# google-deepmind/open_spiel

Hardware: AMD Instinct MI355X
Metric: env-steps/sec (batched LegalActions+ApplyAction+status, connect_four) (higher is better)
Workload: dtype u64; 1 GPU; connect_four fused LegalActions+ApplyAction+status, 2^20 states/GPU, seed 0x5EED; states_per_gpu=1048576, parallelism=1 independent shard(s), no collective

## Files before the change

### open_spiel_amd/csrc/osg_c4_step.h

```cpp
#ifndef OSG_C4_STEP_H_
#define OSG_C4_STEP_H_

#include "osg_common.h"

namespace osg {

OSG_HD uint64_t c4_fours(uint64_t b) {
  uint64_t hit, m;
  m = b & (b >> 1); hit = m & (m >> 2);
  m = b & (b >> 7); hit |= m & (m >> 14);
  m = b & (b >> 6); hit |= m & (m >> 12);
  m = b & (b >> 8); hit |= m & (m >> 16);
  return hit;
}

OSG_HD uint32_t c4_open_columns(uint32_t all_lo, uint32_t all_hi) {
  const uint32_t tl = (~all_lo >> 5) & 0x00204081u;
  const uint32_t th = (~all_hi >> 1) & 0x00004081u;
  const uint32_t ml = tl * ((1u << 21) | (1u << 15) | (1u << 9) | (1u << 3));
  const uint32_t mh = th * ((1u << 14) | (1u << 8) | (1u << 2));
  return ((ml >> 21) & 0xFu) | (((mh >> 14) & 0x7u) << 4);
}

OSG_HD uint32_t c4_fused_step(uint64_t& x, uint64_t& o, uint32_t a) {
  const uint32_t flags = static_cast<uint32_t>(x >> 56);
  const uint64_t X = x & ((1ull << 56) - 1ull), O = o;
  const uint64_t all = X | O;
  const uint32_t stones = static_cast<uint32_t>(__builtin_popcountll(all));
  const uint32_t mover = stones & 1u;
  const bool valid = a < 7u;
  const uint32_t sh = valid ? a * 7u : 0u;
  const uint64_t cell = (all + (1ull << sh)) & (0x3Full << sh);
  const bool apply = valid & ((flags & 1u) == 0u) & (cell != 0ull);
  const uint64_t put = apply ? cell : 0ull;
  const uint64_t to_x = mover ? 0ull : ~0ull;
  const uint64_t nx = X | (put & to_x), no = O | (put & ~to_x);
  const uint64_t b = mover ? no : nx;
  const bool win = c4_fours(b) != 0ull;
  const uint32_t stones_after = stones + (apply ? 1u : 0u);
  const bool done = win | (stones_after == 42u);
  const uint32_t fresh = done ? (((win ? mover : 2u) << 1) | 1u) : 0u;
  const uint32_t nflags = apply ? fresh : flags;
  const uint64_t nall = nx | no;
  const uint32_t open = c4_open_columns(static_cast<uint32_t>(nall), static_cast<uint32_t>(nall >> 32));
  const bool over = (nflags & 1u) != 0u;
  const uint32_t st_run = (stones_after & 1u) + 1u;
  const uint32_t st_over = 0x80u | (nflags >> 1);
  const uint32_t st = (over ? st_over : st_run) | (((a != 0xFFu) & !apply) ? 0x40u : 0u);
  x = nx | (static_cast<uint64_t>(nflags) << 56);
  o = no;
  return (over ? 0u : open) | (st << 8);
}

}
#endif
```

### open_spiel_amd/csrc/osg_step.hip

```cpp
#include "osg_batch_internal.h"
#include "osg_c4_step.h"
#include "osg_ttt_step.h"

namespace {

OSG_D uint8_t encode_status(bool terminal, bool illegal, int cur, int outcome) {
  uint8_t v = illegal ? 0x40 : 0;
  if (terminal) return v | 0x80 | static_cast<uint8_t>(outcome & 7);
  return v | static_cast<uint8_t>((cur + 1) & 15);
}
template <class G> struct has_fused_step : std::false_type {};
template <int R, int C, int K, class BB> struct has_fused_step<C4T<R, C, K, BB>> : std::integral_constant<bool, !C4T<R, C, K, BB>::kStored> {};
template <class G, typename MaskT>
__global__ void __launch_bounds__(kBlock)
k_step(typename G::Params p, const typename G::word_t* src, typename G::word_t* dst, int64_t n,
       const uint8_t* actions, MaskT* mask_out, int mask_elems, uint8_t* status) {
  int64_t i = static_cast<int64_t>(blockIdx.x) * kBlock + threadIdx.x;
  if (i >= n) return;
  typename G::State s = G::load(p, src, n, i);
  int a = actions[i];
  if constexpr (has_fused_step<G>::value) {
    bool illegal_f, term_f;
    int outcome_f;
    const uint32_t open = G::fused_step(p, s, a, illegal_f, term_f, outcome_f);
    G::store(p, dst, n, i, s);
    if (sizeof(MaskT) < 4) {
      mask_out[i] = static_cast<MaskT>(open);
    } else {
#pragma unroll
      for (int w = 0; w < G::kMaskW; ++w)
        if (w < mask_elems) mask_out[i * mask_elems + w] = static_cast<MaskT>(w == 0 ? open : 0u);
    }
    status[i] = encode_status(term_f, illegal_f, term_f ? 0 : (G::plies(s) & 1), term_f ? outcome_f : 0);
    return;
  }
  bool illegal = false;
  if (a != 0xFF) {
    auto before = G::legal(p, s);
    if (a < 32 * G::kMaskW && before.test(a)) G::apply(p, s, a); else illegal = true;
  }
  G::store(p, dst, n, i, s);
  bool term = G::terminal(p, s);
  auto after = G::legal(p, s);
  if (sizeof(MaskT) < 4) {
    mask_out[i] = static_cast<MaskT>(after.w[0]);
  } else {
#pragma unroll
    for (int w = 0; w < G::kMaskW; ++w)
      if (w < mask_elems) mask_out[i * mask_elems + w] = static_cast<MaskT>(after.w[w]);
  }
  status[i] = encode_status(term, illegal, term ? 0 : G::current_player(p, s), term ? G::outcome_code(p, s) : 0);
}

template <class G, typename MaskT, int V, int W>
__global__ void __launch_bounds__(kBlock)
k_step_vec(typename G::Params p, const typename G::word_t* src, typename G::word_t* dst, int64_t n,
           const uint8_t* __restrict__ actions, MaskT* __restrict__ mask_out, uint8_t* __restrict__ status) {
  using word_t = typename G::word_t;
  typedef word_t wvec __attribute__((ext_vector_type(V)));
  typedef uint8_t bvec __attribute__((ext_vector_type(V)));
  typedef MaskT mvec __attribute__((ext_vector_type(V)));
  const int64_t i = (static_cast<int64_t>(blockIdx.x) * kBlock + threadIdx.x) * V;
  if (i >= n) return;
  word_t tmp[W * V];
#pragma unroll
  for (int w = 0; w < W; ++w) {
    const wvec v = *reinterpret_cast<const wvec*>(src + w * n + i);
#pragma unroll
    for (int j = 0; j < V; ++j) tmp[w * V + j] = v[j];
  }
  const bvec av = *reinterpret_cast<const bvec*>(actions + i);
  bvec sv;
  mvec mv;
#pragma unroll
  for (int j = 0; j < V; ++j) {
    if constexpr (std::is_same<G, Ttt>::value) {
      const uint32_t r = ttt_fused_step(tmp[j], av[j]);
      mv[j] = static_cast<MaskT>(r & 0xFFFFu);
      sv[j] = static_cast<uint8_t>(r >> 16);
      continue;
    }
    typename G::State s = G::load(p, tmp, V, j);
    const int a = av[j];
    bool illegal = false;
    if (a != 0xFF) {
      const auto before = G::legal(p, s);
      if (a < 32 * G::kMaskW && before.test(a)) G::apply(p, s, a); else illegal = true;
    }
    G::store(p, tmp, V, j, s);
    const bool term = G::terminal(p, s);
    const auto after = G::legal(p, s);
    mv[j] = static_cast<MaskT>(after.w[0]);
    sv[j] = encode_status(term, illegal, term ? 0 : G::current_player(p, s), term ? G::outcome_code(p, s) : 0);
  }
#pragma unroll
  for (int w = 0; w < W; ++w) {
    wvec v;
#pragma unroll
    for (int j = 0; j < V; ++j) v[j] = tmp[w * V + j];
    __builtin_nontemporal_store(v, reinterpret_cast<wvec*>(dst + w * n + i));
  }
  __builtin_nontemporal_store(mv, reinterpret_cast<mvec*>(mask_out + i));
  __builtin_nontemporal_store(sv, reinterpret_cast<bvec*>(status + i));
}

template <int NW, int V, bool kNt, bool kMask = true, bool kFold = false>
__global__ void __launch_bounds__(kBlock)
k_step_hexvec(typename HexT<NW>::Params p, const uint32_t* src, uint32_t* dst, int64_t n,
              const uint8_t* __restrict__ actions, uint32_t* __restrict__ mask_out, uint8_t* __restrict__ status) {
  using G = HexT<NW>;
  constexpr int W = kFold ? 4 * NW : 4 * NW + 1;
  typedef uint32_t wvec __attribute__((ext_vector_type(V)));
  typedef uint8_t bvec __attribute__((ext_vector_type(V)));
  const int64_t i = (static_cast<int64_t>(blockIdx.x) * kBlock + threadIdx.x) * V;
  if (i >= n) return;
  uint32_t tmp[W * V];
#pragma unroll
  for (int w = 0; w < W; ++w) {
    const wvec v = *reinterpret_cast<const wvec*>(src + w * n + i);
#pragma unroll
    for (int j = 0; j < V; ++j) tmp[w * V + j] = v[j];
  }
  const bvec av = *reinterpret_cast<const bvec*>(actions + i);
  uint32_t mk[NW * V];
  bvec sv;
#pragma unroll
  for (int j = 0; j < V; ++j) {
    typename G::State s = G::template load_as<kFold>(tmp, V, j);
    const int a = av[j];
    bool illegal = false;
    if (a != 0xFF) {
      const auto before = G::legal(p, s);
      if (a < 32 * G::kMaskW && before.test(a)) G::apply(p, s, a); else illegal = true;
    }
    G::template store_as<kFold>(tmp, V, j, s);
    const bool term = G::terminal(p, s);
    if constexpr (kMask) {
      const auto after = G::legal(p, s);
#pragma unroll
      for (int w = 0; w < NW; ++w) mk[j * NW + w] = after.w[w];
    }
    sv[j] = encode_status(term, illegal, term ? 0 : G::current_player(p, s), term ? G::outcome_code(p, s) : 0);
  }
#pragma unroll
  for (int w = 0; w < W; ++w) {
    wvec v;
#pragma unroll
    for (int j = 0; j < V; ++j) v[j] = tmp[w * V + j];
    if constexpr (kNt) __builtin_nontemporal_store(v, reinterpret_cast<wvec*>(dst + w * n + i));
    else *reinterpret_cast<wvec*>(dst + w * n + i) = v;
  }
  if constexpr (kMask) {
#pragma unroll
    for (int k = 0; k < NW; ++k) {
      wvec v;
#pragma unroll
      for (int j = 0; j < V; ++j) v[j] = mk[k * V + j];
      if constexpr (kNt) __builtin_nontemporal_store(v, reinterpret_cast<wvec*>(mask_out + i * NW) + k);
      else reinterpret_cast<wvec*>(mask_out + i * NW)[k] = v;
    }
  }
  if constexpr (kNt) __builtin_nontemporal_store(sv, reinterpret_cast<bvec*>(status + i));
  else *reinterpret_cast<bvec*>(status + i) = sv;
}

constexpr int kC4StepBlock = 128;
template <class G>
__global__ void __launch_bounds__(kC4StepBlock)
k_step_c4x2(typename G::Params p, const uint64_t* src, uint64_t* dst, int64_t n,
            const uint8_t* __restrict__ actions, uint8_t* __restrict__ mask_out, uint8_t* __restrict__ status) {
  const int64_t pair = static_cast<int64_t>(blockIdx.x) * kC4StepBlock + threadIdx.x;
  const int64_t i = pair * 2;
  if (i >= n) return;
  const ulonglong2 xs = *reinterpret_cast<const ulonglong2*>(src + i);
  const ulonglong2 os = *reinterpret_cast<const ulonglong2*>(src + n + i);
  const uint32_t a2 = *reinterpret_cast<const uint16_t*>(actions + i);
  uint64_t x[2] = {xs.x, xs.y}, o[2] = {os.x, os.y};
  uint32_t m2 = 0, s2 = 0;
#pragma unroll
  for (int j = 0; j < 2; ++j) {
    typename G::State s = G::unpack(x[j], o[j]);
    const int a = (a2 >> (8 * j)) & 0xFF;
    bool term = G::terminal(p, s);
    bool illegal = false;
    if (a != 0xFF) {
      if (!term && G::column_has_room(p, s, a)) {
        G::apply(p, s, a);
        term = G::terminal(p, s);
      } else {
        illegal = true;
      }
    }
    const uint32_t open = G::open_columns(p, s);
    const int to_move = G::plies(s) & 1;
    x[j] = G::pack0(s);
    o[j] = s.o;
    m2 |= (term ? 0u : (open & 0xFFu)) << (8 * j);
    s2 |= static_cast<uint32_t>(encode_status(term, illegal, to_move, term ? G::outcome_code(p, s) : 0)) << (8 * j);
  }
  *reinterpret_cast<ulonglong2*>(dst + i) = make_ulonglong2(x[0], x[1]);
  *reinterpret_cast<ulonglong2*>(dst + n + i) = make_ulonglong2(o[0], o[1]);
  *reinterpret_cast<uint16_t*>(mask_out + i) = static_cast<uint16_t>(m2);
  *reinterpret_cast<uint16_t*>(status + i) = static_cast<uint16_t>(s2);
}

__global__ void __launch_bounds__(kC4StepBlock)
k_step_c4std(const uint64_t* src, uint64_t* dst, int64_t n, const uint8_t* __restrict__ actions,
             uint8_t* __restrict__ mask_out, uint8_t* __restrict__ status) {
  const int64_t i = static_cast<int64_t>(blockIdx.x) * kC4StepBlock + threadIdx.x;
  if (i >= n) return;
  uint64_t x = src[i], o = src[n + i];
  const uint32_t r = c4_fused_step(x, o, actions[i]);
  __builtin_nontemporal_store(x, dst + i);
  __builtin_nontemporal_store(o, dst + n + i);
  __builtin_nontemporal_store(static_cast<uint8_t>(r), mask_out + i);
  __builtin_nontemporal_store(static_cast<uint8_t>(r >> 8), status + i);
}

__global__ void __launch_bounds__(kC4StepBlock)
k_step_c4std2(const uint64_t* src, uint64_t* dst, int64_t n, const uint8_t* __restrict__ actions,
              uint8_t* __restrict__ mask_out, uint8_t* __restrict__ status) {
  const int64_t i = (static_cast<int64_t>(blockIdx.x) * kC4StepBlock + threadIdx.x) * 2;
  if (i >= n) return;
  typedef uint64_t u64x2 __attribute__((ext_vector_type(2)));
  typedef uint8_t u8x2 __attribute__((ext_vector_type(2)));
  const u64x2 xs = *reinterpret_cast<const u64x2*>(src + i), os = *reinterpret_cast<const u64x2*>(src + n + i);
  const u8x2 av = *reinterpret_cast<const u8x2*>(actions + i);
  uint64_t x0 = xs.x, x1 = xs.y, o0 = os.x, o1 = os.y;
  const uint32_t r0 = c4_fused_step(x0, o0, av.x), r1 = c4_fused_step(x1, o1, av.y);
  u64x2 xo, oo;
  xo.x = x0; xo.y = x1; oo.x = o0; oo.y = o1;
  u8x2 mo, so;
  mo.x = static_cast<uint8_t>(r0); mo.y = static_cast<uint8_t>(r1);
  so.x = static_cast<uint8_t>(r0 >> 8); so.y = static_cast<uint8_t>(r1 >> 8);
  __builtin_nontemporal_store(xo, reinterpret_cast<u64x2*>(dst + i));
  __builtin_nontemporal_store(oo, reinterpret_cast<u64x2*>(dst + n + i));
  __builtin_nontemporal_store(mo, reinterpret_cast<u8x2*>(mask_out + i));
  __builtin_nontemporal_store(so, reinterpret_cast<u8x2*>(status + i));
}

}

extern "C" {

int osg_step(const osg_batch* src, osg_batch* dst, const uint8_t* d_actions, void* d_mask, uint8_t* d_status) {
  if (!same_game(dst, src) || dst->n != src->n) return set_error(OSG_ERR_INVALID, "osg_step: shape mismatch");
  if (src->spec.desc.num_distinct_actions > 255)
    return set_error(OSG_ERR_UNSUPPORTED, "osg_step: action ids travel as one byte here (0xFF = skip); games with more than 255 "
                                          "actions (hex above 15 x 15) step through osg_apply / osg_env_step (32-bit actions)");
  osg_ctx* ctx = dst->ctx;
  const int cmb = src->spec.desc.compact_mask_bytes;
  const int W = src->spec.desc.mask_words;
  const int64_t n = src->n;
  if (!d_mask && !(src->spec.desc.game_kind == kHex && W == src->spec.hex_nw && W <= 4))
    return set_error(OSG_ERR_UNSUPPORTED, "osg_step: d_mask may be NULL only for hex boards of up to 128 cells (there the successor's "
                                          "mask is ~occupied of the record written); every other game's mask comes from the step itself");
  const bool planes16 = ((reinterpret_cast<uintptr_t>(src->words()) | reinterpret_cast<uintptr_t>(dst->words())) & 15u) == 0;
  if (planes16 && src->spec.desc.game_kind == kC4 && src->spec.c4_std && (n & 1) == 0 &&
      ((reinterpret_cast<uintptr_t>(d_actions) | reinterpret_cast<uintptr_t>(d_mask) | reinterpret_cast<uintptr_t>(d_status)) & 1u) == 0) {
    k_step_c4std2<<<dim3(static_cast<unsigned>((n / 2 + kC4StepBlock - 1) / kC4StepBlock)), dim3(kC4StepBlock), 0, ctx->stream>>>(
        static_cast<const uint64_t*>(src->words()), static_cast<uint64_t*>(dst->words()), n, d_actions,
        static_cast<uint8_t*>(d_mask), d_status);
    OSG_HIP(hipGetLastError());
    return OSG_OK;
  }
  if (src->spec.desc.game_kind == kC4 && src->spec.c4_std) {
    k_step_c4std<<<dim3(static_cast<unsigned>((n + kC4StepBlock - 1) / kC4StepBlock)), dim3(kC4StepBlock), 0, ctx->stream>>>(
        static_cast<const uint64_t*>(src->words()), static_cast<uint64_t*>(dst->words()), n, d_actions,
        static_cast<uint8_t*>(d_mask), d_status);
    OSG_HIP(hipGetLastError());
    return OSG_OK;
  }
  const bool aligned2 = ((reinterpret_cast<uintptr_t>(d_actions) | reinterpret_cast<uintptr_t>(d_mask) |
                          reinterpret_cast<uintptr_t>(d_status)) & 1u) == 0;
  if (planes16 && src->spec.desc.game_kind == kC4 && !src->spec.c4_wide && (n & 1) == 0 && aligned2) {
    const int64_t pairs = n / 2;
    k_step_c4x2<C4><<<dim3(static_cast<unsigned>((pairs + kC4StepBlock - 1) / kC4StepBlock)), dim3(kC4StepBlock), 0, ctx->stream>>>(
        src->spec.c4, static_cast<const uint64_t*>(src->words()), static_cast<uint64_t*>(dst->words()), n, d_actions,
        static_cast<uint8_t*>(d_mask), d_status);
    OSG_HIP(hipGetLastError());
    return OSG_OK;
  }
  const uintptr_t side = reinterpret_cast<uintptr_t>(d_actions) | reinterpret_cast<uintptr_t>(d_mask) | reinterpret_cast<uintptr_t>(d_status);
  const int kind = src->spec.desc.game_kind;
  if (planes16 && kind == kTtt && (n & 3) == 0 && (side & 7u) == 0 && cmb == 2) {
    k_step_vec<Ttt, uint16_t, 4, 1><<<dim3(grid_for(n / 4)), dim3(kBlock), 0, ctx->stream>>>(
        src->spec.ttt, static_cast<const uint32_t*>(src->words()), static_cast<uint32_t*>(dst->words()), n, d_actions,
        static_cast<uint16_t*>(d_mask), d_status);
    OSG_HIP(hipGetLastError());
    return OSG_OK;
  }
  if (planes16 && kind == kKuhn && (n & 1) == 0 && (side & 1u) == 0 && cmb == 1) {
    k_step_vec<Kuhn, uint8_t, 2, 1><<<dim3(grid_for(n / 2)), dim3(kBlock), 0, ctx->stream>>>(
        src->spec.kuhn, static_cast<const uint64_t*>(src->words()), static_cast<uint64_t*>(dst->words()), n, d_actions,
        static_cast<uint8_t*>(d_mask), d_status);
    OSG_HIP(hipGetLastError());
    return OSG_OK;
  }
  if (planes16 && kind == kLeduc && !src->spec.leduc_big && n >= (int64_t{1} << 22) && (n & 1) == 0 && (side & 1u) == 0 && cmb == 1) {
    k_step_vec<Leduc, uint8_t, 2, 2><<<dim3(grid_for(n / 2)), dim3(kBlock), 0, ctx->stream>>>(
        src->spec.leduc, static_cast<const uint64_t*>(src->words()), static_cast<uint64_t*>(dst->words()), n, d_actions,
        static_cast<uint8_t*>(d_mask), d_status);
    OSG_HIP(hipGetLastError());
    return OSG_OK;
  }
  if (kind == kHex && (cmb == 4 * W || !d_mask) && W == src->spec.hex_nw && W <= 4) {
    int v = 2, nt = n >= (int64_t{1} << 22) ? 1 : 0;
    if (const char* e = std::getenv("OSG_HEX_STEP")) {
      int ev = 0, ent = 0;
      if (std::sscanf(e, "%d:%d", &ev, &ent) == 2 && (ev == 1 || ev == 2)) { v = ev; nt = ent ? 1 : 0; }
    }
    while (v > 1 && ((n % v) != 0 || (side & static_cast<uintptr_t>(v - 1)) != 0 ||
                     (reinterpret_cast<uintptr_t>(d_mask) & static_cast<uintptr_t>(4 * v - 1)) != 0 || !planes16))
      v >>= 1;
    if (v > 1) {
      const auto* s32 = static_cast<const uint32_t*>(src->words());
      auto* d32 = static_cast<uint32_t*>(dst->words());
      auto* m32 = static_cast<uint32_t*>(d_mask);
      if (int rc = for_hex(src->spec, [&](auto nw, const auto& P) -> int {
            constexpr int NW = decltype(nw)::value;
            if constexpr (NW <= 4) {
              return with_bool(src->spec.hex_fold, [&](auto fold) {
                return with_bool(nt != 0, [&](auto ntv) {
                  return with_bool(m32 != nullptr, [&](auto mask) {
                    k_step_hexvec<NW, 2, decltype(ntv)::value, decltype(mask)::value, decltype(fold)::value>
                        <<<dim3(grid_for(n / 2)), dim3(kBlock), 0, ctx->stream>>>(P, s32, d32, n, d_actions, m32, d_status);
                    return OSG_OK;
                  });
                });
              });
            }
            return OSG_OK;
          })) return rc;
      OSG_HIP(hipGetLastError());
      return OSG_OK;
    }
  }
  if (!d_mask)
    return set_error(OSG_ERR_UNSUPPORTED, "osg_step: d_mask may be NULL only for hex boards of up to 128 cells stepped two states per "
                                          "thread (an even batch, 2-byte aligned side arrays): there the successor's mask is ~occupied "
                                          "of the record written; every other game's mask is computed by the step itself");
  const auto step = [&](auto m, int mask_stride) {
    using M = decltype(m);
    return for_game(src->spec, [&](auto g, const auto& P) {
      using G = typename decltype(g)::type;
      k_step<G, M><<<dim3(grid_for(n)), dim3(kBlock), 0, ctx->stream>>>(P, static_cast<const typename G::word_t*>(src->words()),
          static_cast<typename G::word_t*>(dst->words()), n, d_actions,
          static_cast<M*>(d_mask), mask_stride, d_status);
      return OSG_OK;
    });
  };
  if (int rc = cmb == 1 ? step(uint8_t{}, 1) : cmb == 2 ? step(uint16_t{}, 1) : step(uint32_t{}, W)) return rc;
  OSG_HIP(hipGetLastError());
  return OSG_OK;
}

}
```

Baseline: 228.2 billion env-steps/s.

## Step two connect-four states per thread with packed 16-bit high-word bitboard math

Adds a paired fused-step path that splits each 64-bit bitboard into 32-bit halves and packs the two states' small upper words into one register. Four-in-a-row detection then runs on the packed word using packed 16-bit shifts, alignbit funnels, perm and bitop3, and the mask and status bytes are extracted with perm. A fallback to the scalar path handles boards whose high bits exceed 16, and an asm hint keeps the kernel pointers in scalar registers. The goal is fewer 64-bit ALU instructions in a kernel that may be memory-bound, at the cost of more complex code and a divergent branch.

```diff
diff --git a/open_spiel_amd/csrc/osg_c4_step.h b/open_spiel_amd/csrc/osg_c4_step.h
--- a/open_spiel_amd/csrc/osg_c4_step.h
+++ b/open_spiel_amd/csrc/osg_c4_step.h
@@ -52,5 +52,134 @@
   return (over ? 0u : open) | (st << 8);
 }
 
+
+typedef uint16_t c4_u16x2 __attribute__((ext_vector_type(2)));
+
+OSG_HD uint32_t c4_pk_shr(uint32_t p, uint32_t d) {
+  const c4_u16x2 v = __builtin_bit_cast(c4_u16x2, p) >> static_cast<uint16_t>(d);
+  return __builtin_bit_cast(uint32_t, v);
+}
+OSG_HD uint32_t c4_funnel(uint32_t hi, uint32_t lo, uint32_t d) {
+#if defined(__HIP_DEVICE_COMPILE__)
+  return __builtin_amdgcn_alignbit(hi, lo, d);
+#else
+  return (lo >> d) | (hi << (32u - d));
+#endif
+}
+OSG_HD uint32_t c4_pack16(uint32_t lo, uint32_t hi) {
+#if defined(__HIP_DEVICE_COMPILE__)
+  return __builtin_amdgcn_perm(hi, lo, 0x05040100u);
+#else
+  return (lo & 0xFFFFu) | (hi << 16);
+#endif
+}
+OSG_HD uint32_t c4_upper16(uint32_t lo, uint32_t hi) {
+#if defined(__HIP_DEVICE_COMPILE__)
+  return __builtin_amdgcn_perm(hi, lo, 0x07060302u);
+#else
+  return (lo >> 16) | (hi & 0xFFFF0000u);
+#endif
+}
+constexpr uint32_t kA = 0xF0u, kB = 0xCCu, kC = 0xAAu;
+template <uint32_t T> OSG_HD uint32_t c4_op3(uint32_t a, uint32_t b, uint32_t c) {
+#if defined(__HIP_DEVICE_COMPILE__)
+  return __builtin_amdgcn_bitop3_b32(a, b, c, T & 0xFFu);
+#else
+  uint32_t r = 0u;
+  for (uint32_t k = 0; k < 8u; ++k)
+    if ((T >> k) & 1u) r |= ((k & 4u) ? a : ~a) & ((k & 2u) ? b : ~b) & ((k & 1u) ? c : ~c);
+  return r;
+#endif
+}
+OSG_HD uint32_t c4_select(uint32_t m, uint32_t a, uint32_t b) { return c4_op3<(kA & kB) | (~kA & kC)>(m, a, b); }
+OSG_HD uint32_t c4_andn_or(uint32_t a, uint32_t b, uint32_t c) { return c4_op3<(kA & ~kB) | kC>(a, b, c); }
+
+struct c4_placement {
+  uint32_t put_lo, put_hi, tx, stones_after, flags;
+  bool apply;
+};
+OSG_HD c4_placement c4_place(uint32_t x_lo, uint32_t x_hi_raw, uint32_t o_lo, uint32_t o_hi, uint32_t a) {
+  c4_placement r;
+  r.flags = x_hi_raw >> 24;
+  const uint32_t all_lo = x_lo | o_lo, all_hi = (x_hi_raw & 0xFFFFFFu) | o_hi;
+  const uint32_t stones = static_cast<uint32_t>(__builtin_popcount(all_lo) + __builtin_popcount(all_hi));
+  const bool ok = (a < 7u) & ((r.flags & 1u) == 0u);
+  const uint32_t sh = (a * 7u) & 63u;
+  const uint32_t col = static_cast<uint32_t>(((static_cast<uint64_t>(all_hi) << 32) | all_lo) >> sh);
+  const uint32_t cell = (col + 1u) & (ok ? 0x3Fu : 0u);
+  const uint64_t put = static_cast<uint64_t>(cell) << sh;
+  r.apply = cell != 0u;
+  r.put_lo = static_cast<uint32_t>(put);
+  r.put_hi = static_cast<uint32_t>(put >> 32);
+  r.tx = (stones & 1u) - 1u;
+  r.stones_after = stones + (r.apply ? 1u : 0u);
+  return r;
+}
+
+OSG_HD uint32_t c4_finish(const c4_placement& p, bool win, uint32_t open, uint32_t a, uint32_t& nflags) {
+  const uint32_t mover = (p.tx & 1u) ^ 1u;
+  const bool done = win | (p.stones_after == 42u);
+  const uint32_t fresh = done ? (((win ? mover : 2u) << 1) | 1u) : 0u;
+  nflags = p.apply ? fresh : p.flags;
+  const bool over = (nflags & 1u) != 0u;
+  const uint32_t st_run = (p.stones_after & 1u) + 1u;
+  const uint32_t st_over = 0x80u | (nflags >> 1);
+  const uint32_t st = (over ? st_over : st_run) | (((a != 0xFFu) & !p.apply) ? 0x40u : 0u);
+  return (over ? 0u : open) | (st << 8);
+}
+
+template <uint32_t D>
+OSG_HD void c4_fours_dir(uint32_t b0, uint32_t b1, uint32_t bp, uint32_t bh1, uint32_t& h0, uint32_t& h1, uint32_t& hp) {
+  const uint32_t mp = bp & c4_pk_shr(bp, D);
+  const uint32_t m0 = b0 & c4_funnel(bp, b0, D), m1 = b1 & c4_funnel(bh1, b1, D);
+  h0 |= m0 & c4_funnel(mp, m0, 2u * D);
+  if constexpr (2u * D < 16u) {
+    hp |= mp & c4_pk_shr(mp, 2u * D);
+    h1 |= m1 & c4_funnel(mp >> 16, m1, 2u * D);
+  } else {
+    h1 |= m1 & c4_upper16(m1, mp);
+  }
+}
+
+OSG_HD uint32_t c4_fused_step_pair(uint64_t& x0, uint64_t& o0, uint32_t a0, uint64_t& x1, uint64_t& o1, uint32_t a1) {
+  const uint32_t xl0 = static_cast<uint32_t>(x0), xr0 = static_cast<uint32_t>(x0 >> 32);
+  const uint32_t ol0 = static_cast<uint32_t>(o0), oh0 = static_cast<uint32_t>(o0 >> 32);
+  const uint32_t xl1 = static_cast<uint32_t>(x1), xr1 = static_cast<uint32_t>(x1 >> 32);
+  const uint32_t ol1 = static_cast<uint32_t>(o1), oh1 = static_cast<uint32_t>(o1 >> 32);
+  if (((((xr0 | xr1) & 0xFFFFFFu) | oh0 | oh1) >> 16) != 0u) {
+    const uint32_t r0 = c4_fused_step(x0, o0, a0), r1 = c4_fused_step(x1, o1, a1);
+    return r0 | (r1 << 16);
+  }
+  const c4_placement p0 = c4_place(xl0, xr0, ol0, oh0, a0), p1 = c4_place(xl1, xr1, ol1, oh1, a1);
+  const uint32_t nxl0 = xl0 | (p0.put_lo & p0.tx), nol0 = c4_andn_or(p0.put_lo, p0.tx, ol0);
+  const uint32_t nxl1 = xl1 | (p1.put_lo & p1.tx), nol1 = c4_andn_or(p1.put_lo, p1.tx, ol1);
+  const uint32_t bl0 = c4_select(p0.tx, nxl0, nol0), bl1 = c4_select(p1.tx, nxl1, nol1);
+  const uint32_t txp = c4_select(0xFFFF0000u, p1.tx, p0.tx);
+  const uint32_t putp = c4_pack16(p0.put_hi, p1.put_hi);
+  const uint32_t nxp = c4_pack16(xr0, xr1) | (putp & txp);
+  const uint32_t nop = c4_andn_or(putp, txp, oh0 | (oh1 << 16));
+  const uint32_t bp = c4_select(txp, nxp, nop);
+  const uint32_t bh1 = bp >> 16;
+  uint32_t hit0 = 0u, hit1 = 0u, hitp = 0u;
+  c4_fours_dir<1>(bl0, bl1, bp, bh1, hit0, hit1, hitp);
+  c4_fours_dir<7>(bl0, bl1, bp, bh1, hit0, hit1, hitp);
+  c4_fours_dir<6>(bl0, bl1, bp, bh1, hit0, hit1, hitp);
+  c4_fours_dir<8>(bl0, bl1, bp, bh1, hit0, hit1, hitp);
+  const bool win0 = (hit0 | (hitp & 0xFFFFu)) != 0u, win1 = (hit1 | (hitp & 0xFFFF0000u)) != 0u;
+  const uint32_t roomp = ~(nxp | nop);
+  const uint32_t tl0 = (~(nxl0 | nol0) >> 5) & 0x00204081u, tl1 = (~(nxl1 | nol1) >> 5) & 0x00204081u;
+  const uint32_t th0 = (roomp >> 1) & 0x00004081u, th1 = (roomp >> 17) & 0x00004081u;
+  const uint32_t kL = (1u << 21) | (1u << 15) | (1u << 9) | (1u << 3), kH = (1u << 14) | (1u << 8) | (1u << 2);
+  const uint32_t open0 = (((tl0 * kL) >> 21) & 0xFu) | ((((th0 * kH) >> 14) & 0x7u) << 4);
+  const uint32_t open1 = (((tl1 * kL) >> 21) & 0xFu) | ((((th1 * kH) >> 14) & 0x7u) << 4);
+  uint32_t nf0, nf1;
+  const uint32_t r0 = c4_finish(p0, win0, open0, a0, nf0), r1 = c4_finish(p1, win1, open1, a1, nf1);
+  x0 = nxl0 | (static_cast<uint64_t>((nxp & 0xFFFFu) | (nf0 << 24)) << 32);
+  x1 = nxl1 | (static_cast<uint64_t>((nxp >> 16) | (nf1 << 24)) << 32);
+  o0 = nol0 | (static_cast<uint64_t>(nop & 0xFFFFu) << 32);
+  o1 = nol1 | (static_cast<uint64_t>(nop >> 16) << 32);
+  return r0 | (r1 << 16);
+}
+
 }
 #endif
diff --git a/open_spiel_amd/csrc/osg_step.hip b/open_spiel_amd/csrc/osg_step.hip
--- a/open_spiel_amd/csrc/osg_step.hip
+++ b/open_spiel_amd/csrc/osg_step.hip
@@ -221,18 +221,18 @@
 k_step_c4std2(const uint64_t* src, uint64_t* dst, int64_t n, const uint8_t* __restrict__ actions,
               uint8_t* __restrict__ mask_out, uint8_t* __restrict__ status) {
   const int64_t i = (static_cast<int64_t>(blockIdx.x) * kC4StepBlock + threadIdx.x) * 2;
+  asm volatile("" ::"s"(src), "s"(dst), "s"(actions), "s"(mask_out), "s"(status));
   if (i >= n) return;
   typedef uint64_t u64x2 __attribute__((ext_vector_type(2)));
   typedef uint8_t u8x2 __attribute__((ext_vector_type(2)));
   const u64x2 xs = *reinterpret_cast<const u64x2*>(src + i), os = *reinterpret_cast<const u64x2*>(src + n + i);
   const u8x2 av = *reinterpret_cast<const u8x2*>(actions + i);
   uint64_t x0 = xs.x, x1 = xs.y, o0 = os.x, o1 = os.y;
-  const uint32_t r0 = c4_fused_step(x0, o0, av.x), r1 = c4_fused_step(x1, o1, av.y);
+  const uint32_t r = c4_fused_step_pair(x0, o0, av.x, x1, o1, av.y);
   u64x2 xo, oo;
   xo.x = x0; xo.y = x1; oo.x = o0; oo.y = o1;
-  u8x2 mo, so;
-  mo.x = static_cast<uint8_t>(r0); mo.y = static_cast<uint8_t>(r1);
-  so.x = static_cast<uint8_t>(r0 >> 8); so.y = static_cast<uint8_t>(r1 >> 8);
+  const u8x2 mo = __builtin_bit_cast(u8x2, static_cast<uint16_t>(__builtin_amdgcn_perm(0u, r, 0x0c0c0200u)));
+  const u8x2 so = __builtin_bit_cast(u8x2, static_cast<uint16_t>(__builtin_amdgcn_perm(0u, r, 0x0c0c0301u)));
   __builtin_nontemporal_store(xo, reinterpret_cast<u64x2*>(dst + i));
   __builtin_nontemporal_store(oo, reinterpret_cast<u64x2*>(dst + n + i));
   __builtin_nontemporal_store(mo, reinterpret_cast<u8x2*>(mask_out + i));
```

Result: slower. 225.4 billion env-steps/s (-1.2%).
